# liuQuan98/APR

Measured on AMD Instinct MI355X. Metric: point-cloud pairs/sec (120k-pt KITTI frame, FCGF encode+match+SVD), higher is better.
Workload: dtype f32

## Files before the change

### apr_amd/_lib.py

```python
from __future__ import annotations

import ctypes as C
import os

import torch

_HERE = os.path.dirname(os.path.abspath(__file__))
LIB_PATH = os.path.join(_HERE, "lib", "libapr_hip.so")

_p = C.c_void_p
_i32, _i64, _u64, _f32, _f64, _sz = C.c_int32, C.c_int64, C.c_uint64, C.c_float, C.c_double, C.c_size_t

class PairDesc(C.Structure):
    _fields_ = [("f0", C.c_void_p), ("n0", C.c_int64), ("f1", C.c_void_p), ("n1", C.c_int64),
                ("xyz0", C.c_void_p), ("xyz1", C.c_void_p), ("seed", C.c_uint64)]


class SpconvDesc(C.Structure):
    _fields_ = [("inp", C.c_void_p), ("ldi", C.c_int64), ("nbr", C.c_void_p), ("n_out", C.c_int64),
                ("K", C.c_int32), ("cin", C.c_int32), ("cout", C.c_int32), ("relu", C.c_int32),
                ("w_packed", C.c_void_p), ("scale", C.c_void_p), ("shift", C.c_void_p),
                ("residual", C.c_void_p), ("ldr", C.c_int64), ("out", C.c_void_p), ("ldo", C.c_int64),
                ("counters", C.c_void_p), ("plist", C.c_void_p), ("prod_scratch", C.c_void_p),
                ("plist_bytes", C.c_int64), ("w_bf3", C.c_void_p),
# ... 86 lines not shown
    "apr_pairlist3_build": (C.c_int, [_p, _i64, _i32, _p, _p, _sz, _p]),
    "apr_spconv_ws3_supported": (C.c_int, [_i32, _i32, _i32]),
    "apr_spconv_ws3_fwd_bf3": (C.c_int, [_p, _i64, _p, _p, _i64, _i32, _i32, _p, _p, _p, _p, _i64, _i32, _p, _i64, _p, _p]),
    "apr_spconv_ws_fwd": (C.c_int, [_p, _i64, _p, _p, _i64, _i32, _i32, _i32, _p, _p, _p, _p, _i64, _i32, _p, _i64, _p, _p]),
    "apr_spconv_packed_bf3_bytes": (_i64, [_i32, _i32, _i32]),
    "apr_spconv_pack_weights_bf3": (C.c_int, [_p, _i32, _i32, _i32, _p, _p]),
    "apr_spconv_pack_weights_bf3_ex": (C.c_int, [_p, _i32, _i32, _i32, _i32, _i32, _p, _p]),
    "apr_spconv_ws_fwd_bf3": (C.c_int, [_p, _i64, _p, _p, _i64, _i32, _i32, _i32, _p, _p, _p, _p, _p, _i64, _i32, _p, _i64,
                                        _p, _p]),
    "apr_spconv_wgrad_scratch_bytes": (_sz, [_i64, _i32, _i32, _i32]),
    "apr_spconv_wgrad": (C.c_int, [_p, _i64, _p, _i64, _p, _i64, _i32, _i32, _i32, _p, _p, _sz, _p]),
    "apr_spconv_wgrad_same_level": (C.c_int, [_p, _i64, _p, _i64, _p, _i64, _i32, _i32, _i32, _p, _p, _sz, _p]),
    "apr_spconv_route": (_i32, [_p]),
    "apr_spconv_tile_variant": (_i32, [_p]),
    "apr_dense_gemm_bf3_variant": (_i32, [_i64, _i32, _i32]),
    "apr_spconv_wgrad_plan": (C.c_int, [_p, _i64, _p, _i64, _i64, _i32, _i32, _i32, _i32, _p]),
    "apr_spconv_ws_supported": (_i32, [_i32, _i32, _i32]),
    "apr_spconv_bigk_supported": (_i32, [_i32, _i32, _i32]),
    "apr_spconv_fwd_batch": (C.c_int, [_p, _i32, _p]),
    "apr_spconv_fwd_batch_timed": (C.c_int, [_p, _i32, _p, _p]),
    "apr_bn_stats": (C.c_int, [_p, _i64, _i64, _i32, _p, _p, _p, _sz, _p]),
    "apr_norm_params": (C.c_int, [_p, _i64, _i64, _i32, _f32, _p, _p, _p, _sz, _p]),
    "apr_bn_stats_scratch_bytes": (_sz, [_i64, _i32]),
    "apr_instance_norm_act": (C.c_int, [_p, _i64, _i64, _i32, _f32, _p, _i64, _i32, _f32, _p, _i64, _p, _sz, _p]),
    "apr_spconv_os_tile_rows": (_i32, [_i64, _i32, _i32]),
    "apr_spconv_os_pairs_bytes": (_sz, [_i64, _i32, _i32]),
    "apr_spconv_os_pairs_build": (C.c_int, [_p, _i64, _i64, _i32, _i32, _p, _sz, _p]),
    "apr_spconv_os_trace": (C.c_int, [_p, _i32]),
    "apr_spconv_os_set_debug": (C.c_int, [_i32]),
    "apr_spconv_os_fwd": (C.c_int, [_p, _i64, _p, _i64, _i32, _i32, _i32, _i32, _p, _p, _p, _p, _i64, _i32, _p, _i64, _p]),
    "apr_norm_backward_scratch_bytes": (_sz, [_i64, _i32]),
    "apr_norm_backward": (C.c_int, [_p, _i64, _p, _i64, _i64, _i32, _p, _p, _p, _p, _i64, _p, _p, _p, _sz, _p]),
    "apr_bn_train_fwd": (C.c_int, [_p, _i64, _i64, _i32, _p, _p, C.c_float, C.c_float, _p, _p, _p, _i64, _i32, _p, _i64, _p, _p,
                                   _p, _p, _i32, _p, _sz, _p]),
    "apr_bn_train_bwd": (C.c_int, [_p, _i64, _p, _i64, _p, _i64, _i64, _i32, _p, _p, _p, _i32, _p, _i64, _p, _i64, _p, _p,
                                   _p, _i32, _p, _sz, _p]),
    "apr_weights_flip_transpose": (C.c_int, [_p, _i32, _i32, _i32, _i32, _p, _p]),
    "apr_dense_gemm_bf3": (C.c_int, [_p, _i64, _i64, _i32, _i32, _p, _p, _p, _p, _i64, _i32, _p, _i64, _p]),
    "apr_dense_rows_bf3_ok": (_i32, [_i32, _i32]),
    "apr_dense_rows_bf3_route": (_i32, [_i64, _i32, _i32]),
    "apr_dense_rows_bf3": (C.c_int, [_p, _i64, _i64, _i32, _i32, _p, _p, _p, _p, _i64, _i32, _i32, _p, _i64, _p]),
    "apr_dense_gemm_bf3_norm_scratch_bytes": (_sz, [_i64, _i32, _i32]),
    "apr_dense_gemm_bf3_norm_act": (C.c_int, [_p, _i64, _i64, _i32, _i32, _p, _f32, _p, _i64, _i32, _f32, _p, _i64, _p, _i32, _p,
                                              _sz, _p]),
    "apr_weighted_choice_round": (C.c_int64, [_p, _i64, _p, _i64, _i64, _p, _i64, _p, _p, _i32]),
    "apr_instance_norm_act_seg": (C.c_int, [_p, _i64, _i64, _i32, _f32, _p, _i64, _i32, _f32, _p, _i64, _p, _i32, _p, _sz, _p]),
    "apr_affine_act": (C.c_int, [_p, _i64, _i64, _i32, _p, _p, _p, _i64, _i32, _f32, _p, _i64, _p]),
    "apr_act_backward": (C.c_int, [_p, _i64, _p, _i64, _i64, _i32, _i32, _f32, _p, _i64, _p]),
    "apr_l2_normalize": (C.c_int, [_p, _i64, _i64, _i32, _p, _i64, _p]),
    "apr_l2_normalize_backward": (C.c_int, [_p, _i64, _p, _i64, _i64, _i32, _p, _i64, _p]),
    "apr_feature_nn": (C.c_int, [_p, _i64, _p, _i64, _i32, _p, _p]),
    "apr_feature_nn_fast_scratch_bytes": (_sz, [_i64, _i64, _i32]),
    "apr_feature_nn_fast": (C.c_int, [_p, _i64, _p, _i64, _i32, _p, _p, _sz, _p]),
    "apr_nn_unpack": (C.c_int, [_p, _i64, _p, _p, _p]),
    "apr_ransac_scratch_bytes": (_sz, [_i64, _i64]),
    "apr_ransac_pose": (C.c_int, [_p, _i64, _p, _i64, _p, _f64, _f64, _i64, _u64, _p, _sz, _p, _p]),
    "apr_ransac_geometric_scratch_bytes": (_sz, [_i64, _i64, _i64]),
    "apr_ransac_pose_geometric": (C.c_int, [_p, _i64, _p, _i64, _p, _f64, _f64, _i64, _i64, _u64, _p, _sz, _p, _p]),
    "apr_ransac_raw_bytes": (_sz, []),
    "apr_ransac_pose_geometric_async": (C.c_int, [_p, _i64, _p, _i64, _p, _f64, _f64, _i64, _i64, _u64, _p, _sz, _p, _p]),
    "apr_ransac_decode": (C.c_int, [_p, _p]),
    "apr_ransac_pose_async": (C.c_int, [_p, _i64, _p, _i64, _p, _f64, _f64, _i64, _u64, _p, _sz, _p, _p]),
    "apr_fcgf_test_pair": (C.c_int, [_p, _i64, _p, _i64, _p, _p, _i64, _i64, _p, _p, _i64, _p, _i64, _p, _p, _p, _f64, _f64,
                                     _f64, _i64, _p, _p, _i64, _i64, _p]),
    "apr_irls_pose": (C.c_int, [_p, _p, _p, _i64, _p, _p, _sz, _p]),
    "apr_match_pose_batch_scratch_bytes": (_sz, [_i32, _i64, _i64, _i32, _i64]),
    "apr_match_pose_batch": (C.c_int, [_p, _i32, _i32, C.c_double, C.c_double, _i64, _p, _sz, _p, _p]),
    "apr_match_pose_batch_slot_bytes": (_sz, [_i32]),
    "apr_match_pose_set_lanes": (C.c_int, [_i32]),
    "apr_match_pose_batch_enqueue": (C.c_int, [_p, _i32, _i32, C.c_double, C.c_double, _i64, _p, _sz, _p, _p]),
    "apr_match_pose_batch_finish": (C.c_int, [_p, _i32, _i32, C.c_double, C.c_double, _i64, _p, _sz, _p, _p, _p]),
    "apr_irls_scratch_bytes": (_sz, [_i64]),
    "apr_valid_pair": (C.c_int, [_p, _i64, _p, _i64, _p, _p, _i64, _i64, _p, _p, _f32, _p, _i64, _i64, _p, _sz, _p]),
    "apr_valid_pair_scratch_bytes": (_sz, [_i64]),
    "apr_predator_valid_record": (C.c_int, [_p, _p, _p, _p, _p, _p, _p, _p, _i64, _i64, _p, _i64, _i64, _p]),
    "apr_predator_test_pair": (C.c_int, [_p, _i64, _p, _i64, _p, _p, _p, _p, _f64, _f64, _f64, _f64, _p, _i64, _i64, _p]),
    "apr_contrastive_reduce": (C.c_int, [_p, _p, _i32, _i32, _p, _p, _p, _p, _p, _p, _p, _i32, _i64, _f32, _f32, _p, _p]),
    "apr_pair_rows_from_nn": (C.c_int, [_p, _i64, _p, _i64, _p, _p]),
    "apr_pair_dist": (C.c_int, [_p, _i64, _p, _i64, _i32, _p, _p, _i64, _i64, _f32, _p, _p, _p, _p]),
    "apr_pair_terms_scratch_bytes": (_sz, [_i64]),
    "apr_pair_terms_reduce": (C.c_int, [_p, _p, _p, _i64, _p, _i64, _p, _i64, _i64, _f32, _i32, _p, _p, _p, _p, _p, _p, _sz, _p]),
    "apr_pair_grad_scratch_bytes": (_sz, [_i64, _i64, _i64]),
    "apr_pair_grad": (C.c_int, [_p, _i64, _p, _i64, _i32, _p, _p, _i64, _p, _p, _p, _p, _i32, _p, _p, _p, _sz, _p]),
    "apr_grid_subsample_scratch_bytes": (_sz, [_i64]),
    "apr_grid_subsample": (C.c_int, [_p, _i64, _p, _i32, _f32, _p, _i32, _p, _p, _p, _p, _sz, _p]),
    "apr_grid_subsample_async": (C.c_int, [_p, _i64, _p, _i32, _f32, _p, _i32, _p, _p, _p, _p, _sz, _p]),
    "apr_voxel_down_sample_scratch_bytes": (_sz, [_i64]),
    "apr_voxel_down_sample": (C.c_int, [_p, _i64, _p, _i32, _f64, _p, _p, _p, _p, _p, _p, _p, _sz, _p]),
    "apr_sample_augment": (C.c_int, [_p, _p, _i64, _f64, _p, _f64, _p, _p, _p]),
    "apr_cloud_mean": (C.c_int, [_p, _i64, _p, _p]),
    "apr_radius_scratch_bytes": (_sz, [_i64, _i64]),
    "apr_radius_neighbors_async": (C.c_int, [_p, _i64, _p, _i64, _p, _p, _i32, _f32, _i32, _p, _i64, _p, _p, _sz, _p]),
    "apr_radius_neighbors_regrid_async": (C.c_int, [_p, _i64, _p, _i64, _p, _p, _i32, _f32, _i32, _p, _i64, _p, _p, _sz, _p]),
    "apr_radius_neighbors": (C.c_int, [_p, _i64, _p, _i64, _p, _p, _i32, _f32, _i32, _p, _i64, _p, _p, _sz, _p]),
    "apr_knn": (C.c_int, [_p, _i32, _i32, _i32, _p, _p]),
    "apr_row_sums": (C.c_int, [_p, _i64, _i64, _i32, _p, _p]),
    "apr_kpconv_weighted": (C.c_int, [_p, _i64, _p, _i64, _p, _i32, _p, _i64, _i32, _p, _i32, _f32, _p, _p, _i64, _p]),
    "apr_kpconv_fused_ok": (_i32, [_i32, _i32, _i32]),
    "apr_kpconv_fused_route": (_i32, [_i64, _i32, _i32, _i32]),
    "apr_kpconv_fused": (C.c_int, [_p, _i64, _p, _i64, _p, _i32, _p, _i64, _i32, _p, _i32, _f32, _p, _p, _i32, _p, _i64, _p]),
    "apr_kpconv_dfeat": (C.c_int, [_p, _i64, _p, _i64, _p, _i32, _p, _i64, _i32, _p, _i32, _f32, _p, _p, _i64, _p]),
    "apr_kpconv_dfeat_contrib": (C.c_int, [_p, _i64, _p, _i64, _p, _i32, _p, _i64, _i32, _p, _i32, _f32, _p, _p, _p]),
    "apr_kpconv_deform_weighted": (C.c_int, [_p, _i64, _p, _i64, _p, _i32, _p, _i64, _i32, _p, _p, _i32, _f32, _p, _p, _i64, _p,
                                             _p]),
    "apr_kpconv_deform_dfeat_contrib": (C.c_int, [_p, _i64, _p, _i64, _p, _i32, _p, _i64, _i32, _p, _p, _i32, _f32, _p, _p, _p]),
    "apr_kpconv_deform_dgeom": (C.c_int, [_p, _i64, _p, _i64, _p, _i32, _p, _i64, _i32, _p, _i64, _p, _p, _i32, _f32, _p, _p, _p,
# ... 130 lines not shown
```

### apr_amd/csrc/match_mfma.hip

```cpp
#include "common.h"

namespace {

typedef float f32x4 __attribute__((ext_vector_type(4)));
typedef float f32x2 __attribute__((ext_vector_type(2)));
typedef __bf16 bf16x8 __attribute__((ext_vector_type(8)));

constexpr float kEpsRel = 1e-4f;
constexpr float kEpsAbs = 5e-5f;

__device__ inline unsigned short to_bf16_rne(float x) {
  unsigned u = __float_as_uint(x);
  u += 0x7FFFu + ((u >> 16) & 1u);
  return (unsigned short)(u >> 16);
}

template <int C>
__global__ void k_nn_prep(const float* __restrict__ f, int64_t n, float len_scale, float row_scale,
                          unsigned short* __restrict__ fb, unsigned short* __restrict__ fl, f32x4* __restrict__ meta,
                          unsigned* __restrict__ u_init, unsigned long long* __restrict__ best_init,
                          unsigned* __restrict__ zero_me) {
  constexpr int LPR = C / 4;
  const int64_t t = (int64_t)blockIdx.x * blockDim.x + threadIdx.x;
  const int64_t row = t / LPR;
// ... 315 lines not shown
    }
  }
  if (!REFINE && wave_live) {
#pragma unroll
    for (int qt = 0; qt < QT; ++qt)
#pragma unroll
      for (int r = 0; r < 4; ++r) {
        float v = mn[qt][r];
#pragma unroll
        for (int d = 1; d < 16; d <<= 1) v = fminf(v, __shfl_xor(v, d));
        const int64_t row = q0 + qt * 16 + lq * 4 + r;
        if (l16 == 0 && row < n0) {
          const f32x4 m = qmeta[row];
          const float u = fmaxf(v + m[1] + m[0] * len_max, 0.f);
          atomicMin(&U[row], __float_as_uint(u));
        }
      }
  }
}

template <int C>
__device__ inline void nn_tile_eval(float* my_t, const f32x4* xv, const float* __restrict__ f1, int64_t j0, int64_t j1,
                                    int lane, float& bd, int& bj) {
  constexpr int VPR = C / 4;
#pragma unroll
  for (int v = lane; v < 16 * VPR; v += 64) {
    const int r = v / VPR, g = v - r * VPR;
    const int64_t row = (j0 + r < j1) ? j0 + r : j1 - 1;
    *reinterpret_cast<f32x4*>(my_t + r * C + g * 4) = *reinterpret_cast<const f32x4*>(f1 + row * C + g * 4);
  }
#pragma unroll 2
  for (int jj = 0; jj < 16; ++jj) {
    float s0 = 0.f, s1 = 0.f, s2 = 0.f, s3 = 0.f;
#pragma unroll
    for (int g = 0; g < C / 4; ++g) {
      const f32x4 yv = *reinterpret_cast<const f32x4*>(my_t + jj * C + g * 4);
      const float d0 = xv[g][0] - yv[0], d1 = xv[g][1] - yv[1];
      const float d2 = xv[g][2] - yv[2], d3 = xv[g][3] - yv[3];
      s0 = fmaf(d0, d0, s0);
      s1 = fmaf(d1, d1, s1);
      s2 = fmaf(d2, d2, s2);
      s3 = fmaf(d3, d3, s3);
    }
    const float dd = (s0 + s1) + (s2 + s3);
    const int64_t j = (j0 + jj < j1) ? j0 + jj : j1 - 1;
    if (dd < bd) {
      bd = dd;
      bj = (int)j;
    }
  }
}

template <int C>
__global__ __launch_bounds__(256) void k_nn_resolve(const unsigned long long* __restrict__ cand,
                                                    const unsigned* __restrict__ cand_count, unsigned nwg, unsigned nexact,
                                                    const unsigned long long* __restrict__ shared_list,
                                                    const unsigned* __restrict__ overflow, unsigned shared_cap,
                                                    const unsigned* __restrict__ dense_list, int chunk, unsigned qwaves,
                                                    const float* __restrict__ f0, int64_t n0,
                                                    const float* __restrict__ f1, int64_t n1,
                                                    unsigned long long* __restrict__ best) {
  __shared__ __attribute__((aligned(16))) float s_t[4][16 * C];
  const int lane = threadIdx.x & 63;
  const int wave = __builtin_amdgcn_readfirstlane(threadIdx.x >> 6);
  if (overflow[0] != 0u) {
    const int64_t nqt = (n0 + 63) >> 6, ntt = (n1 + 15) >> 4;
    const int64_t nw = (int64_t)gridDim.x * 4;
    const int64_t slices = nw / nqt > 0 ? nw / nqt : 1;
    const int64_t tps = (ntt + slices - 1) / slices;
    for (int64_t w = (int64_t)blockIdx.x * 4 + wave; w < nqt * slices; w += nw) {
      const int64_t q = (w % nqt) * 64 + lane;
      const int64_t tt0 = (w / nqt) * tps, tt1 = min((long long)(tt0 + tps), (long long)ntt);
      const float* x = f0 + (q < n0 ? q : n0 - 1) * C;
      f32x4 xv[C / 4];
#pragma unroll
      for (int g = 0; g < C / 4; ++g) xv[g] = *reinterpret_cast<const f32x4*>(x + g * 4);
      float bd = __builtin_inff();
      int bj = 0x7fffffff;
      for (int64_t tt = tt0; tt < tt1; ++tt)
        nn_tile_eval<C>(s_t[wave], xv, f1, tt * 16, min((long long)(tt * 16 + 16), (long long)n1), lane, bd, bj);
      if (q < n0 && bj != 0x7fffffff) {
        const unsigned long long mine = ((unsigned long long)__float_as_uint(bd) << 32) | (unsigned)bj;
        if (mine < __builtin_nontemporal_load(&best[q])) atomicMin(&best[q], mine);
      }
    }
    return;
  }
  if (blockIdx.x < nexact) {
    const bool shared = blockIdx.x >= nwg;
    const unsigned wave_id = blockIdx.x * 4 + (threadIdx.x >> 6);
    const unsigned n = shared ? min(overflow[1], shared_cap) : min(cand_count[wave_id], (unsigned)kCandWave);
    const unsigned long long* src = shared ? shared_list : cand + (size_t)wave_id * kCandWave;
    const unsigned first = shared ? (blockIdx.x - nwg) * 256u + threadIdx.x : (threadIdx.x & 63u);
    const unsigned step = shared ? (nexact - nwg) * 256u : 64u;
    for (unsigned t = first; t < n; t += step) {
      const unsigned long long ij = src[t];
      const int64_t i = (int64_t)(ij >> 32), j = (int64_t)(ij & 0xffffffffull);
      const float* x = f0 + i * C;
      const float* y = f1 + j * C;
      float s0 = 0.f, s1 = 0.f, s2 = 0.f, s3 = 0.f;
#pragma unroll
      for (int g = 0; g < C / 4; ++g) {
        const f32x4 xv = *reinterpret_cast<const f32x4*>(x + g * 4);
        const f32x4 yv = *reinterpret_cast<const f32x4*>(y + g * 4);
        const float d0 = xv[0] - yv[0], d1 = xv[1] - yv[1], d2 = xv[2] - yv[2], d3 = xv[3] - yv[3];
        s0 = fmaf(d0, d0, s0);
        s1 = fmaf(d1, d1, s1);
        s2 = fmaf(d2, d2, s2);
        s3 = fmaf(d3, d3, s3);
      }
      const float d = (s0 + s1) + (s2 + s3);
      const unsigned long long mine = ((unsigned long long)__float_as_uint(d) << 32) | (unsigned)j;
      if (mine < __builtin_nontemporal_load(&best[i])) atomicMin(&best[i], mine);
    }
    return;
  }
  const unsigned tpc = (unsigned)chunk >> 4;
  const unsigned n = min(overflow[2], kDenseListCap);
  const unsigned nwaves = (gridDim.x - nexact) * 4;
  for (unsigned e = (blockIdx.x - nexact) * 4 + wave; e < n; e += nwaves) {
    const unsigned fb = __builtin_amdgcn_readfirstlane(dense_list[e]);
    const unsigned wave_id = fb / tpc, tile = fb % tpc;
    const unsigned dq = (wave_id % qwaves) * 64u;
    const unsigned t0 = (wave_id / qwaves) * (unsigned)chunk;
    const int64_t q = (int64_t)dq + lane;
    const int64_t j0 = (int64_t)t0 + (int64_t)tile * 16;
    const int64_t j1 = min(min((long long)(j0 + 16), (long long)((int64_t)t0 + chunk)), (long long)n1);
    const float* x = f0 + (q < n0 ? q : n0 - 1) * C;
    f32x4 xv[C / 4];
#pragma unroll
    for (int g = 0; g < C / 4; ++g) xv[g] = *reinterpret_cast<const f32x4*>(x + g * 4);
    float bd = __builtin_inff();
    int bj = 0x7fffffff;
    nn_tile_eval<C>(s_t[wave], xv, f1, j0, j1, lane, bd, bj);
    if (q < n0 && bj != 0x7fffffff) {
      const unsigned long long mine = ((unsigned long long)__float_as_uint(bd) << 32) | (unsigned)bj;
      if (mine < __builtin_nontemporal_load(&best[q])) atomicMin(&best[q], mine);
    }
  }
}

int64_t shared_capacity(int64_t n0) {
  int64_t c = 64 * n0;
  if (c < 65536) c = 65536;
  return c < (1ll << 31) ? c : (1ll << 31) - 1;
}

void nn_grid(int64_t n0, int64_t n1, int feat_c, int64_t* qblocks, int64_t* chunk, int64_t* nchunk) {
  static const int s_wgs = env_int("APR_NN_GRID_WGS", 768);
  static const int s_want = env_int("APR_NN_WANT", 0);
  *qblocks = cdiv64(n0, 256);
  int64_t want = cdiv64(s_wgs > 0 && s_wgs < 768 ? s_wgs : 768, *qblocks);
  if (feat_c >= 64) {
    const int64_t fit = 512 / *qblocks;
    if (fit >= 1 && fit < want) want = fit;
  }
  if (s_want > 0 && s_want <= want) want = s_want;
  int64_t c = cdiv64(cdiv64(n1, want), 64) * 64;
  if (c < 256) c = 256;
  if (c >= (1 << 24)) c = (1 << 24) - 64;
  *chunk = c;
  *nchunk = cdiv64(n1, c);
}

size_t dense_list_bytes(int64_t qblocks, int64_t nchunk, int64_t chunk) {
  uint64_t nflag = (uint64_t)(qblocks * 4) * (uint64_t)nchunk * (uint64_t)(chunk / 16);
  if (nflag > kDenseListCap) nflag = kDenseListCap;
  return apr_align256((size_t)nflag * 4 + 64);
}

template <int C>
int run_fast(const float* f0, int64_t n0, const float* f1, int64_t n1, unsigned long long* best, void* scratch,
             size_t scratch_bytes, hipStream_t st) {
  AprArena a(scratch);
  int64_t qblocks, chunk, nchunk;
  nn_grid(n0, n1, C, &qblocks, &chunk, &nchunk);
  const int64_t nwaves = qblocks * nchunk * 4;
  unsigned short* qb = a.take<unsigned short>((size_t)n0 * C);
  unsigned short* ql = a.take<unsigned short>((size_t)n0 * C);
  unsigned short* tb = a.take<unsigned short>((size_t)n1 * C);
  unsigned short* tl = a.take<unsigned short>((size_t)n1 * C);
  f32x4* qmeta = a.take<f32x4>(n0);
  f32x4* tmeta = a.take<f32x4>(n1);
  unsigned* U = a.take<unsigned>(n0);
  unsigned* overflow = a.take<unsigned>(64);
  unsigned* cand_count = a.take<unsigned>(nwaves);
  unsigned long long* cand = a.take<unsigned long long>((size_t)nwaves * kCandWave);
  unsigned long long* shared_list = a.take<unsigned long long>(shared_capacity(n0));
  a.take<char>((size_t)(qblocks * 4) * (size_t)nchunk * (size_t)(chunk / 16) + 64);
  unsigned* dense_list = (unsigned*)a.take<char>(dense_list_bytes(qblocks, nchunk, chunk));
  APR_CHECK_ARG(a.fits(scratch_bytes), "apr_feature_nn_fast: scratch too small");
  const unsigned shared_cap = (unsigned)shared_capacity(n0);
  constexpr int LPR = C / 4;
  if ((uint64_t)qblocks * 4 * (uint64_t)nchunk * (uint64_t)(chunk / 16) + 64 >= (1ull << 32)) {
    apr_set_error("apr_feature_nn_fast: problem too large for the dense-block ids");
    return APR_EINVAL;
  }
  hipLaunchKernelGGL((k_nn_prep2<C>), dim3((unsigned)cdiv64((n0 + n1) * LPR, 256)), dim3(256), 0, st, f0, n0, f1, n1, qb, ql,
                     qmeta, tb, tl, tmeta, U, best, overflow);
  static const int s_dense_min = env_int("APR_NN_DENSE_MIN", kDenseMin);
  static const int s_bound_div = env_int("APR_NN_BOUND_DIV", 4);
  const dim3 grid((unsigned)qblocks, (unsigned)nchunk);
  hipLaunchKernelGGL((k_nn_mfma<C, false>), grid, dim3(256), 0, st, qb, ql, qmeta, n0, tb, tl, tmeta, n1, (int)chunk, U,
                     cand, cand_count, overflow, shared_list, shared_cap, dense_list, overflow + 2, s_bound_div);
  hipLaunchKernelGGL((k_nn_mfma<C, true>), grid, dim3(256), 0, st, qb, ql, qmeta, n0, tb, tl, tmeta, n1, (int)chunk, U,
                     cand, cand_count, overflow, shared_list, shared_cap, dense_list, overflow + 2, s_dense_min);
  const unsigned nwg = (unsigned)(qblocks * nchunk);
  const unsigned nexact = nwg + 256;
  hipLaunchKernelGGL((k_nn_resolve<C>), dim3(nexact + 1024), dim3(256), 0, st, cand, cand_count, nwg, nexact, shared_list,
                     overflow, shared_cap, dense_list, (int)chunk, (unsigned)(qblocks * 4), f0, n0, f1, n1, best);
  APR_LAUNCH_CHECK();
  return APR_OK;
}

}

APR_API size_t apr_feature_nn_fast_scratch_bytes(int64_t n0, int64_t n1, int32_t c) {
  if (n0 < 0 || n1 < 0 || c <= 0) return 0;
  if (n0 < 1) n0 = 1;
  if (n1 < 1) n1 = 1;
  const size_t qblocks = (size_t)cdiv64(n0, 256);
  const size_t nwaves = 4 * (768 + qblocks);
  const size_t nflag = qblocks * 4 * ((2 * (size_t)n1 + 320) / 16 + 1);
  const size_t nlist = nflag > kDenseListCap ? (size_t)kDenseListCap : nflag;
  const auto al = apr_align256;
  return 2 * al((size_t)n0 * c * 2) + 2 * al((size_t)n1 * c * 2) + al((size_t)n0 * 16) + al((size_t)n1 * 16) +
         al((size_t)n0 * 4) + 256 + al(nwaves * 4) + al(nwaves * kCandWave * 8) +
         al((size_t)shared_capacity(n0) * 8) + al(nflag + 64) + al(nlist * 4 + 64) + 512;
}

APR_API int apr_feature_nn_fast(const float* f0, int64_t n0, const float* f1, int64_t n1, int32_t c, uint64_t* best,
                                void* scratch, size_t scratch_bytes, void* stream) {
  hipStream_t st = (hipStream_t)stream;
  APR_CHECK_ARG(n0 >= 0 && n1 > 0 && n1 < (1ll << 31) && n0 < (1ll << 31), "apr_feature_nn_fast: bad shape");
  APR_CHECK_ARG(c == 32 || c == 64 || c == 128, "apr_feature_nn_fast: c=%d, supported: 32, 64, 128", c);
  APR_CHECK_ARG(n1 < (1ll << 24) - 64, "apr_feature_nn_fast: n1 = %lld, supported below 2^24 - 64 targets", (long long)n1);
  APR_CHECK_ARG(((((uintptr_t)f0) | ((uintptr_t)f1)) & 15) == 0, "apr_feature_nn_fast: 16-byte aligned rows required");
  APR_CHECK_ARG(scratch_bytes >= apr_feature_nn_fast_scratch_bytes(n0, n1, c), "apr_feature_nn_fast: scratch too small");
  if (n0 == 0) return APR_OK;
  unsigned long long* b = (unsigned long long*)best;
  if (c == 32) return run_fast<32>(f0, n0, f1, n1, b, scratch, scratch_bytes, st);
  if (c == 64) return run_fast<64>(f0, n0, f1, n1, b, scratch, scratch_bytes, st);
  return run_fast<128>(f0, n0, f1, n1, b, scratch, scratch_bytes, st);
}
```

### apr_amd/ops.py

```python
from __future__ import annotations

import ctypes as C
import os

import numpy as np
import torch

from . import _lib
from ._lib import check, ptr, stream


def _lib_():
    return _lib.load()


def _f32(t, name):
    if not t.is_cuda or t.dtype != torch.float32:
        raise _lib.AprHipError(f"{name}: need a float32 GPU tensor (no CPU fallback), got {t.dtype} on {t.device}")
    return t


def _rows(t, name):
    _f32(t, name)
    if t.dim() != 2 or (t.shape[1] > 1 and t.stride(1) != 1):
# ... 969 lines not shown
    def backward(ctx, dy, _dm, _dv):
        x, mean, rstd, weight = ctx.saved_tensors
        g = None if weight is None else weight.reshape(-1).contiguous()
        dx, dg, db = norm_backward(x, dy.contiguous(), mean, rstd, g, want_affine_grads=weight is not None or ctx.has_bias)
        dw = dg.reshape(weight.shape) if weight is not None else None
        dbias = db if ctx.has_bias else None
        return dx, dw, dbias, None


def affine_act(x, scale=None, shift=None, residual=None, relu=False, out=None, leaky=None):
    x, ldx = _rows(x, "affine_act.x")
    n, c = x.shape
    if out is None:
        out = torch.empty((n, c), dtype=torch.float32, device=x.device)
    out, ldy = _rows(out, "affine_act.out")
    ldr = 0
    if residual is not None:
        residual, ldr = _rows(residual, "affine_act.residual")
    mode = 2 if leaky is not None else int(bool(relu))
    check(_lib_().apr_affine_act(ptr(x), ldx, n, c, ptr(scale), ptr(shift), ptr(residual), ldr, mode,
                                 float(leaky or 0.0), ptr(out), ldy, stream()))
    return out


def l2_normalize(x, out=None):
    x, ldx = _rows(x, "l2_normalize.x")
    n, c = x.shape
    if out is None:
        out = torch.empty((n, c), dtype=torch.float32, device=x.device)
    out, ldy = _rows(out, "l2_normalize.out")
    check(_lib_().apr_l2_normalize(ptr(x), ldx, n, c, ptr(out), ldy, stream()))
    return out


class L2NormalizeFunction(torch.autograd.Function):

    @staticmethod
    def forward(ctx, x):
        x = x.contiguous()
        ctx.save_for_backward(x)
        return l2_normalize(x)

    @staticmethod
    def backward(ctx, dy):
        (x,) = ctx.saved_tensors
        dy = dy.contiguous()
        n, c = x.shape
        dx = torch.empty_like(x)
        check(_lib_().apr_l2_normalize_backward(ptr(x), c, ptr(dy), c, n, c, ptr(dx), c, stream()))
        return dx



def feature_nn(f0, f1, return_distance=False, impl=None):
    f0 = _f32(f0, "feature_nn.f0").contiguous()
    f1 = _f32(f1, "feature_nn.f1").contiguous()
    if f0.shape[1] != f1.shape[1]:
        raise _lib.AprHipError("feature_nn: channel mismatch")
    n0, c = f0.shape
    n1 = f1.shape[0]
    lib = _lib_()
    best = torch.empty(n0, dtype=torch.int64, device=f0.device)
    if impl is None:
        impl = os.environ.get("APR_NN_IMPL", "fast")
    if impl not in ("brute", "fast"):
        raise _lib.AprHipError(f"feature_nn: unknown impl {impl!r}")
    if impl == "fast" and c in (32, 64, 128):
        sb = int(lib.apr_feature_nn_fast_scratch_bytes(n0, n1, c))
        scratch = torch.empty(sb, dtype=torch.uint8, device=f0.device)
        check(lib.apr_feature_nn_fast(ptr(f0), n0, ptr(f1), n1, c, ptr(best), ptr(scratch), sb, stream()))
    else:
        check(lib.apr_feature_nn(ptr(f0), n0, ptr(f1), n1, c, ptr(best), stream()))
    idx = torch.empty(n0, dtype=torch.int64, device=f0.device)
    d2 = torch.empty(n0, dtype=torch.float32, device=f0.device) if return_distance else None
    check(lib.apr_nn_unpack(ptr(best), n0, ptr(idx), ptr(d2), stream()))
    return (idx, d2) if return_distance else idx



def _dev(t, dtype, name):
    if not torch.is_tensor(t) or not t.is_cuda or t.dtype != dtype:
        raise _lib.AprHipError(f"{name}: need a {dtype} GPU tensor (no CPU fallback), got "
                               f"{getattr(t, 'dtype', type(t))} on {getattr(t, 'device', 'the host')}")
    return t.contiguous()


def overlap_labels(correspondence, n_src, n_tgt):
    corr = _dev(correspondence, torch.int64, "overlap_labels.correspondence")
    dev = corr.device
    gt = torch.empty(n_src + n_tgt, dtype=torch.float32, device=dev)
    src_idx = torch.empty(n_src, dtype=torch.int32, device=dev)
    tgt_idx = torch.empty(n_tgt, dtype=torch.int32, device=dev)
    counts = torch.empty(3, dtype=torch.int32, device=dev)
    check(_lib_().apr_overlap_labels(ptr(corr), corr.shape[0], n_src, n_tgt, ptr(gt), ptr(src_idx), ptr(tgt_idx), ptr(counts),
                                     stream()))
    return gt, src_idx, tgt_idx, counts


def weighted_bce(pred, gt, n_dev=None):
    pred, gt = _dev(pred, torch.float32, "weighted_bce.pred"), _dev(gt, torch.float32, "weighted_bce.gt")
    if pred.dim() != 1 or pred.shape != gt.shape:
        raise _lib.AprHipError("weighted_bce: prediction and gt must be vectors of one length")
    lib = _lib_()
    sb = int(lib.apr_weighted_bce_scratch_bytes())
    scratch = torch.empty(sb, dtype=torch.uint8, device=pred.device)
    out = torch.empty(8, dtype=torch.float32, device=pred.device)
    check(lib.apr_weighted_bce_forward(ptr(pred), ptr(gt), pred.shape[0], ptr(n_dev), ptr(out), ptr(scratch), sb, stream()))
    return out


def weighted_bce_backward(pred, gt, out8, grad_out, n_dev=None, scatter_pos=None, dpred=None):
    pred, gt = _dev(pred, torch.float32, "weighted_bce_backward.pred"), _dev(gt, torch.float32, "weighted_bce_backward.gt")
    out8, grad_out = _dev(out8, torch.float32, "weighted_bce_backward.out8"), _dev(grad_out, torch.float32, "weighted_bce_backward.grad_out")
    if dpred is None:
        dpred = torch.zeros_like(pred)
    check(_lib_().apr_weighted_bce_backward(ptr(pred), ptr(gt), pred.shape[0], ptr(n_dev), ptr(out8), ptr(grad_out),
                                            ptr(scatter_pos), ptr(dpred), stream()))
    return dpred


def gathered_argmax(a, a_idx, na_dev, b, b_idx, nb_dev):
    a, b = _dev(a, torch.float32, "gathered_argmax.a"), _dev(b, torch.float32, "gathered_argmax.b")
    a_idx, b_idx = _dev(a_idx, torch.int32, "gathered_argmax.a_idx"), _dev(b_idx, torch.int32, "gathered_argmax.b_idx")
    if a.dim() != 2 or b.dim() != 2 or a.shape[1] != b.shape[1]:
        raise _lib.AprHipError("gathered_argmax: channel mismatch")
    row_arg = torch.zeros(a_idx.shape[0], dtype=torch.int32, device=a.device)
    col_arg = torch.zeros(b_idx.shape[0], dtype=torch.int32, device=a.device)
    check(_lib_().apr_gathered_argmax(ptr(a), ptr(a_idx), ptr(na_dev), a_idx.shape[0], ptr(b), ptr(b_idx), ptr(nb_dev),
                                      b_idx.shape[0], a.shape[1], ptr(row_arg), ptr(col_arg), stream()))
# ... 806 lines not shown
```

### include/apr_hip.h

```cpp
#ifndef APR_HIP_H
#define APR_HIP_H

#include <stddef.h>
#include <stdint.h>

#ifdef __cplusplus
extern "C" {
#endif

#define APR_OK 0
#define APR_EINVAL (-1)
#define APR_EHIP (-2)
#define APR_ETIMEOUT (-3)
#define APR_ERANGE (-3)

const char* apr_last_error(void);
int apr_version(void);
int apr_device_count(void);
int32_t apr_struct_sizes(int32_t* out, int32_t n);
int apr_event_wait(void* event, int32_t poll_us);
int apr_event_wait_timeout(void* event, int32_t poll_us, int64_t timeout_us);


int64_t apr_hash_capacity(int64_t n);
// ... 187 lines not shown
                      void* arena, size_t arena_bytes, apr_pyramid* out, void* stream);


int apr_bn_stats(const float* x, int64_t ld, int64_t n, int32_t c,
                 float* mean, float* var, void* scratch, size_t scratch_bytes, void* stream);
size_t apr_bn_stats_scratch_bytes(int64_t n, int32_t c);

size_t apr_norm_backward_scratch_bytes(int64_t n, int32_t c);
int apr_norm_backward(const float* x, int64_t ldx, const float* dy, int64_t lddy, int64_t n, int32_t c,
                      const float* mean, const float* rstd, const float* gamma, float* dx, int64_t lddx,
                      float* dgamma, float* dbeta, void* scratch, size_t scratch_bytes, void* stream);

int apr_bn_train_fwd(const float* z, int64_t ldz, int64_t n, int32_t c, const float* gamma, const float* beta,
                     float eps, float momentum, float* running_mean, float* running_var, const float* residual,
                     int64_t ldr, int32_t relu, float* y, int64_t ldy, float* save_mean, float* save_rstd,
                     int64_t* num_batches_tracked, const int64_t* seg_offsets_host, int32_t nseg, void* scratch,
                     size_t scratch_bytes, void* stream);
int apr_bn_train_bwd(const float* z, int64_t ldz, const float* y, int64_t ldy, const float* dy, int64_t lddy,
                     int64_t n, int32_t c, const float* mean, const float* rstd, const float* gamma, int32_t relu,
                     float* dx, int64_t lddx, float* dres, int64_t lddres, float* dgamma, float* dbeta,
                     const int64_t* seg_offsets_host, int32_t nseg, void* scratch, size_t scratch_bytes, void* stream);

int apr_col_sums(const float* x, int64_t ld, int64_t n, int32_t c, float* sums, void* scratch, size_t scratch_bytes,
                 void* stream);

int apr_norm_params(const float* x, int64_t ld, int64_t n, int32_t c, float eps, float* scale, float* shift,
                    void* scratch, size_t scratch_bytes, void* stream);

int apr_instance_norm_act(const float* x, int64_t ldx, int64_t n, int32_t c, float eps, const float* residual,
                          int64_t ldr, int32_t relu, float negative_slope, float* y, int64_t ldy, void* scratch,
                          size_t scratch_bytes, void* stream);
int apr_instance_norm_act_seg(const float* x, int64_t ldx, int64_t n, int32_t c, float eps, const float* residual,
                              int64_t ldr, int32_t relu, float negative_slope, float* y, int64_t ldy,
                              const int64_t* seg_offsets_host, int32_t nseg, void* scratch, size_t scratch_bytes,
                              void* stream);

int apr_affine_act(const float* x, int64_t ldx, int64_t n, int32_t c,
                   const float* scale, const float* shift,
                   const float* residual, int64_t ldr, int32_t relu, float negative_slope,
                   float* y, int64_t ldy, void* stream);
int apr_act_backward(const float* dy, int64_t lddy, const float* y, int64_t ldy, int64_t n, int32_t c, int32_t mode,
                     float negative_slope, float* dz, int64_t lddz, void* stream);

int apr_l2_normalize(const float* x, int64_t ldx, int64_t n, int32_t c,
                     float* y, int64_t ldy, void* stream);
int apr_l2_normalize_backward(const float* x, int64_t ldx, const float* dy, int64_t lddy, int64_t n, int32_t c,
                              float* dx, int64_t lddx, void* stream);

int apr_feature_nn(const float* f0, int64_t n0, const float* f1, int64_t n1, int32_t c,
                   uint64_t* best, void* stream);
size_t apr_feature_nn_fast_scratch_bytes(int64_t n0, int64_t n1, int32_t c);
int apr_feature_nn_fast(const float* f0, int64_t n0, const float* f1, int64_t n1, int32_t c, uint64_t* best,
                        void* scratch, size_t scratch_bytes, void* stream);
int apr_nn_unpack(const uint64_t* best, int64_t n, int64_t* idx, float* d2, void* stream);

size_t apr_ransac_scratch_bytes(int64_t n0, int64_t max_iter);
int apr_ransac_pose(const float* xyz0, int64_t n0, const float* xyz1, int64_t n1,
                    const int64_t* corr, double max_dist, double edge_ratio,
                    int64_t max_iter, uint64_t seed,
                    void* scratch, size_t scratch_bytes, double* result_host, void* stream);

size_t apr_ransac_geometric_scratch_bytes(int64_t n0, int64_t n1, int64_t max_iter);
int apr_ransac_pose_geometric(const float* xyz0, int64_t n0, const float* xyz1, int64_t n1,
                              const int64_t* corr, double max_dist, double edge_ratio,
                              int64_t max_iter, int64_t max_validation, uint64_t seed,
                              void* scratch, size_t scratch_bytes, double* result_host, void* stream);
size_t apr_ransac_raw_bytes(void);
int apr_ransac_pose_geometric_async(const float* xyz0, int64_t n0, const float* xyz1, int64_t n1,
                                    const int64_t* corr, double max_dist, double edge_ratio, int64_t max_iter,
                                    int64_t max_validation, uint64_t seed, void* scratch, size_t scratch_bytes,
                                    void* raw_dev, void* stream);
int apr_ransac_decode(const void* raw_host, double* result_host);
int apr_ransac_pose_async(const float* xyz0, int64_t n0, const float* xyz1, int64_t n1, const int64_t* corr,
                          double max_dist, double edge_ratio, int64_t max_iter, uint64_t seed, void* scratch,
                          size_t scratch_bytes, void* raw_dev, void* stream);

typedef struct {
  const float* f0; int64_t n0;
  const float* f1; int64_t n1;
  const float* xyz0;
  const float* xyz1;
  uint64_t seed;
} apr_pair_desc;
size_t apr_match_pose_batch_scratch_bytes(int32_t B, int64_t n0_max, int64_t n1_max, int32_t c, int64_t max_iter);
int apr_match_pose_batch(const apr_pair_desc* pairs, int32_t B, int32_t c, double max_dist, double edge_ratio,
                         int64_t max_iter, void* scratch, size_t scratch_bytes, double* results_host, void* stream);
size_t apr_match_pose_batch_slot_bytes(int32_t B);
int apr_match_pose_batch_enqueue(const apr_pair_desc* pairs, int32_t B, int32_t c, double max_dist, double edge_ratio,
                                 int64_t max_iter, void* scratch, size_t scratch_bytes, void* slots_host, void* stream);
int apr_match_pose_batch_finish(const apr_pair_desc* pairs, int32_t B, int32_t c, double max_dist, double edge_ratio,
                                int64_t max_iter, void* scratch, size_t scratch_bytes, const void* slots_host,
                                double* results_host, void* stream);

int apr_ransac_set_screen(int32_t mode);
int apr_ransac_set_option(int32_t option, int32_t value);
int apr_ransac_sampling_launches(int64_t* out2);

int apr_match_pose_set_lanes(int32_t lanes);

int apr_irls_pose(const float* pts0, const float* pts1, const float* weight, int64_t n,
                  float* T_host, void* scratch, size_t scratch_bytes, void* stream);
size_t apr_irls_scratch_bytes(int64_t n);

#define APR_VALID_RECORD_FLOATS 24
int apr_valid_pair(const float* xyz0, int64_t n0, const float* xyz1, int64_t n1, const int64_t* sel0,
                   const int64_t* sel1, int64_t m0, int64_t m1, const int64_t* nn, const float* T_gt,
// ... 326 lines not shown
```

Baseline: 2783.

## Resolve NN candidates with row-cooperative coalesced loads staged through LDS

Adds a row-cooperative resolve path for the feature nearest-neighbour candidate lists. Lanes now load slices of several candidate rows with coalesced vector loads, write the differences to per-wave LDS, and each lane then reduces one candidate's distance. The old path had one lane gather a whole row on its own. The new path is on by default when a list holds enough candidates. It adds an env override, a counts diagnostic kernel, reusable scratch, and larger LDS use per block, which may lower occupancy.

```diff
diff --git a/apr_amd/_lib.py b/apr_amd/_lib.py
--- a/apr_amd/_lib.py
+++ b/apr_amd/_lib.py
@@ -162,6 +162,7 @@
     "apr_feature_nn": (C.c_int, [_p, _i64, _p, _i64, _i32, _p, _p]),
     "apr_feature_nn_fast_scratch_bytes": (_sz, [_i64, _i64, _i32]),
     "apr_feature_nn_fast": (C.c_int, [_p, _i64, _p, _i64, _i32, _p, _p, _sz, _p]),
+    "apr_feature_nn_fast_counts": (C.c_int, [_p, _i64, _i64, _i32, _p, _p]),
     "apr_nn_unpack": (C.c_int, [_p, _i64, _p, _p, _p]),
     "apr_ransac_scratch_bytes": (_sz, [_i64, _i64]),
     "apr_ransac_pose": (C.c_int, [_p, _i64, _p, _i64, _p, _f64, _f64, _i64, _u64, _p, _sz, _p, _p]),
diff --git a/apr_amd/csrc/match_mfma.hip b/apr_amd/csrc/match_mfma.hip
--- a/apr_amd/csrc/match_mfma.hip
+++ b/apr_amd/csrc/match_mfma.hip
@@ -391,6 +391,89 @@
 }
 
 template <int C>
+__device__ inline void nn_cand_lanes(const unsigned long long* __restrict__ src, unsigned first, unsigned n, unsigned step,
+                                     const float* __restrict__ f0, const float* __restrict__ f1,
+                                     unsigned long long* __restrict__ best) {
+  for (unsigned t = first; t < n; t += step) {
+    const unsigned long long ij = src[t];
+    const int64_t i = (int64_t)(ij >> 32), j = (int64_t)(ij & 0xffffffffull);
+    const float* x = f0 + i * C;
+    const float* y = f1 + j * C;
+    float s0 = 0.f, s1 = 0.f, s2 = 0.f, s3 = 0.f;
+#pragma unroll
+    for (int g = 0; g < C / 4; ++g) {
+      const f32x4 xv = *reinterpret_cast<const f32x4*>(x + g * 4);
+      const f32x4 yv = *reinterpret_cast<const f32x4*>(y + g * 4);
+      const float d0 = xv[0] - yv[0], d1 = xv[1] - yv[1], d2 = xv[2] - yv[2], d3 = xv[3] - yv[3];
+      s0 = fmaf(d0, d0, s0);
+      s1 = fmaf(d1, d1, s1);
+      s2 = fmaf(d2, d2, s2);
+      s3 = fmaf(d3, d3, s3);
+    }
+    const float d = (s0 + s1) + (s2 + s3);
+    const unsigned long long mine = ((unsigned long long)__float_as_uint(d) << 32) | (unsigned)j;
+    if (mine < __builtin_nontemporal_load(&best[i])) atomicMin(&best[i], mine);
+  }
+}
+
+constexpr int kRowsStage = 2048;
+constexpr int kRowsStagePad = kRowsStage + 4 * 64;
+
+template <int C>
+__device__ inline void nn_cand_rows(float* __restrict__ st, const unsigned long long* __restrict__ src, unsigned first,
+                                    unsigned n, unsigned step, const float* __restrict__ f0,
+                                    const float* __restrict__ f1, unsigned long long* __restrict__ best, int lane) {
+  constexpr int LPR = C / 4;
+  constexpr int B = kRowsStage / C;
+  constexpr int RPP = 64 / LPR;
+  constexpr int NP = B / RPP;
+  constexpr int LD = C + 4;
+  const int sub = lane / LPR, g = lane - sub * LPR;
+  if (first >= n) return;
+  auto word = [&](unsigned b0) {
+    const unsigned nb = min(n - b0, (unsigned)B);
+    return src[b0 + min((unsigned)lane, nb - 1u)];
+  };
+  unsigned long long w = word(first);
+  for (unsigned b0 = first; b0 < n; b0 += step) {
+    const unsigned nb = min(n - b0, (unsigned)B);
+    const unsigned wi = (unsigned)(w >> 32), wj = (unsigned)w;
+    f32x4 xv[NP], yv[NP];
+#pragma unroll
+    for (int p = 0; p < NP; ++p) {
+      const int64_t i = (int64_t)(unsigned)__shfl((int)wi, p * RPP + sub);
+      const int64_t j = (int64_t)(unsigned)__shfl((int)wj, p * RPP + sub);
+      xv[p] = *reinterpret_cast<const f32x4*>(f0 + i * C + g * 4);
+      yv[p] = *reinterpret_cast<const f32x4*>(f1 + j * C + g * 4);
+    }
+    const unsigned nxt = b0 + step;
+    unsigned long long wn = 0ull;
+    if (nxt < n) wn = word(nxt);
+    asm volatile("" ::: "memory");
+#pragma unroll
+    for (int p = 0; p < NP; ++p)
+      *reinterpret_cast<f32x4*>(st + (p * RPP + sub) * LD + g * 4) = xv[p] - yv[p];
+    asm volatile("" ::: "memory");
+    if ((unsigned)lane < nb) {
+      const float* d = st + lane * LD;
+      float s0 = 0.f, s1 = 0.f, s2 = 0.f, s3 = 0.f;
+#pragma unroll
+      for (int gg = 0; gg < C / 4; ++gg) {
+        const f32x4 dv = *reinterpret_cast<const f32x4*>(d + gg * 4);
+        s0 = fmaf(dv[0], dv[0], s0);
+        s1 = fmaf(dv[1], dv[1], s1);
+        s2 = fmaf(dv[2], dv[2], s2);
+        s3 = fmaf(dv[3], dv[3], s3);
+      }
+      const float dd = (s0 + s1) + (s2 + s3);
+      const unsigned long long mine = ((unsigned long long)__float_as_uint(dd) << 32) | wj;
+      if (mine < __builtin_nontemporal_load(&best[wi])) atomicMin(&best[wi], mine);
+    }
+    w = wn;
+  }
+}
+
+template <int C, bool ROWS>
 __global__ __launch_bounds__(256) void k_nn_resolve(const unsigned long long* __restrict__ cand,
                                                     const unsigned* __restrict__ cand_count, unsigned nwg, unsigned nexact,
                                                     const unsigned long long* __restrict__ shared_list,
@@ -398,8 +481,10 @@
                                                     const unsigned* __restrict__ dense_list, int chunk, unsigned qwaves,
                                                     const float* __restrict__ f0, int64_t n0,
                                                     const float* __restrict__ f1, int64_t n1,
-                                                    unsigned long long* __restrict__ best) {
-  __shared__ __attribute__((aligned(16))) float s_t[4][16 * C];
+                                                    unsigned long long* __restrict__ best, unsigned rows_min) {
+  constexpr int kWaveLds = ROWS ? kRowsStagePad : 16 * C;
+  static_assert(kWaveLds >= 16 * C && (!ROWS || kWaveLds >= (kRowsStage / C) * (C + 4)), "per-wave LDS too small");
+  __shared__ __attribute__((aligned(16))) float s_t[4][kWaveLds];
   const int lane = threadIdx.x & 63;
   const int wave = __builtin_amdgcn_readfirstlane(threadIdx.x >> 6);
   if (overflow[0] != 0u) {
@@ -430,27 +515,15 @@
     const unsigned wave_id = blockIdx.x * 4 + (threadIdx.x >> 6);
     const unsigned n = shared ? min(overflow[1], shared_cap) : min(cand_count[wave_id], (unsigned)kCandWave);
     const unsigned long long* src = shared ? shared_list : cand + (size_t)wave_id * kCandWave;
-    const unsigned first = shared ? (blockIdx.x - nwg) * 256u + threadIdx.x : (threadIdx.x & 63u);
-    const unsigned step = shared ? (nexact - nwg) * 256u : 64u;
-    for (unsigned t = first; t < n; t += step) {
-      const unsigned long long ij = src[t];
-      const int64_t i = (int64_t)(ij >> 32), j = (int64_t)(ij & 0xffffffffull);
-      const float* x = f0 + i * C;
-      const float* y = f1 + j * C;
-      float s0 = 0.f, s1 = 0.f, s2 = 0.f, s3 = 0.f;
-#pragma unroll
-      for (int g = 0; g < C / 4; ++g) {
-        const f32x4 xv = *reinterpret_cast<const f32x4*>(x + g * 4);
-        const f32x4 yv = *reinterpret_cast<const f32x4*>(y + g * 4);
-        const float d0 = xv[0] - yv[0], d1 = xv[1] - yv[1], d2 = xv[2] - yv[2], d3 = xv[3] - yv[3];
-        s0 = fmaf(d0, d0, s0);
-        s1 = fmaf(d1, d1, s1);
-        s2 = fmaf(d2, d2, s2);
-        s3 = fmaf(d3, d3, s3);
-      }
-      const float d = (s0 + s1) + (s2 + s3);
-      const unsigned long long mine = ((unsigned long long)__float_as_uint(d) << 32) | (unsigned)j;
-      if (mine < __builtin_nontemporal_load(&best[i])) atomicMin(&best[i], mine);
+    if (ROWS && n >= rows_min) {
+      constexpr unsigned B = kRowsStage / C;
+      const unsigned first = shared ? ((blockIdx.x - nwg) * 4u + (unsigned)wave) * B : 0u;
+      const unsigned step = shared ? (nexact - nwg) * 4u * B : B;
+      nn_cand_rows<C>(s_t[wave], src, first, n, step, f0, f1, best, lane);
+    } else {
+      const unsigned first = shared ? (blockIdx.x - nwg) * 256u + threadIdx.x : (threadIdx.x & 63u);
+      const unsigned step = shared ? (nexact - nwg) * 256u : 64u;
+      nn_cand_lanes<C>(src, first, n, step, f0, f1, best);
     }
     return;
   }
@@ -508,26 +581,69 @@
   return apr_align256((size_t)nflag * 4 + 64);
 }
 
+struct NnScratch {
+  int64_t qblocks, chunk, nchunk, nwaves;
+  unsigned short *qb, *ql, *tb, *tl;
+  f32x4 *qmeta, *tmeta;
+  unsigned *U, *overflow, *cand_count, *dense_list;
+  unsigned long long *cand, *shared_list;
+};
+
+NnScratch nn_carve(AprArena& a, int64_t n0, int64_t n1, int c) {
+  NnScratch s;
+  nn_grid(n0, n1, c, &s.qblocks, &s.chunk, &s.nchunk);
+  s.nwaves = s.qblocks * s.nchunk * 4;
+  s.qb = a.take<unsigned short>((size_t)n0 * c);
+  s.ql = a.take<unsigned short>((size_t)n0 * c);
+  s.tb = a.take<unsigned short>((size_t)n1 * c);
+  s.tl = a.take<unsigned short>((size_t)n1 * c);
+  s.qmeta = a.take<f32x4>(n0);
+  s.tmeta = a.take<f32x4>(n1);
+  s.U = a.take<unsigned>(n0);
+  s.overflow = a.take<unsigned>(64);
+  s.cand_count = a.take<unsigned>(s.nwaves);
+  s.cand = a.take<unsigned long long>((size_t)s.nwaves * kCandWave);
+  s.shared_list = a.take<unsigned long long>(shared_capacity(n0));
+  a.take<char>((size_t)(s.qblocks * 4) * (size_t)s.nchunk * (size_t)(s.chunk / 16) + 64);
+  s.dense_list = (unsigned*)a.take<char>(dense_list_bytes(s.qblocks, s.nchunk, s.chunk));
+  return s;
+}
+
+__global__ __launch_bounds__(256) void k_nn_counts(const unsigned* __restrict__ cand_count, int64_t nwaves,
+                                                   const unsigned* __restrict__ overflow, unsigned shared_cap,
+                                                   unsigned long long* __restrict__ counts) {
+  __shared__ unsigned long long s_sum[4];
+  unsigned long long s = 0;
+  for (int64_t w = threadIdx.x; w < nwaves; w += 256) s += min(cand_count[w], (unsigned)kCandWave);
+#pragma unroll
+  for (int d = 32; d >= 1; d >>= 1) s += __shfl_xor(s, d);
+  if ((threadIdx.x & 63) == 0) s_sum[threadIdx.x >> 6] = s;
+  __syncthreads();
+  if (threadIdx.x == 0) {
+    counts[0] = (s_sum[0] + s_sum[1]) + (s_sum[2] + s_sum[3]);
+    counts[1] = min(overflow[1], shared_cap);
+    counts[2] = overflow[2];
+  }
+}
+
+bool nn_resolve_rows() {
+  static const bool s_rows = [] {
+    const char* v = getenv("APR_NN_RESOLVE");
+    return !(v && strcmp(v, "lanes") == 0);
+  }();
+  return s_rows;
+}
+
 template <int C>
 int run_fast(const float* f0, int64_t n0, const float* f1, int64_t n1, unsigned long long* best, void* scratch,
              size_t scratch_bytes, hipStream_t st) {
   AprArena a(scratch);
-  int64_t qblocks, chunk, nchunk;
-  nn_grid(n0, n1, C, &qblocks, &chunk, &nchunk);
-  const int64_t nwaves = qblocks * nchunk * 4;
-  unsigned short* qb = a.take<unsigned short>((size_t)n0 * C);
-  unsigned short* ql = a.take<unsigned short>((size_t)n0 * C);
-  unsigned short* tb = a.take<unsigned short>((size_t)n1 * C);
-  unsigned short* tl = a.take<unsigned short>((size_t)n1 * C);
-  f32x4* qmeta = a.take<f32x4>(n0);
-  f32x4* tmeta = a.take<f32x4>(n1);
-  unsigned* U = a.take<unsigned>(n0);
-  unsigned* overflow = a.take<unsigned>(64);
-  unsigned* cand_count = a.take<unsigned>(nwaves);
-  unsigned long long* cand = a.take<unsigned long long>((size_t)nwaves * kCandWave);
-  unsigned long long* shared_list = a.take<unsigned long long>(shared_capacity(n0));
-  a.take<char>((size_t)(qblocks * 4) * (size_t)nchunk * (size_t)(chunk / 16) + 64);
-  unsigned* dense_list = (unsigned*)a.take<char>(dense_list_bytes(qblocks, nchunk, chunk));
+  const NnScratch s = nn_carve(a, n0, n1, C);
+  const int64_t qblocks = s.qblocks, chunk = s.chunk, nchunk = s.nchunk;
+  unsigned short *qb = s.qb, *ql = s.ql, *tb = s.tb, *tl = s.tl;
+  f32x4 *qmeta = s.qmeta, *tmeta = s.tmeta;
+  unsigned *U = s.U, *overflow = s.overflow, *cand_count = s.cand_count, *dense_list = s.dense_list;
+  unsigned long long *cand = s.cand, *shared_list = s.shared_list;
   APR_CHECK_ARG(a.fits(scratch_bytes), "apr_feature_nn_fast: scratch too small");
   const unsigned shared_cap = (unsigned)shared_capacity(n0);
   constexpr int LPR = C / 4;
@@ -546,8 +662,16 @@
                      cand, cand_count, overflow, shared_list, shared_cap, dense_list, overflow + 2, s_dense_min);
   const unsigned nwg = (unsigned)(qblocks * nchunk);
   const unsigned nexact = nwg + 256;
-  hipLaunchKernelGGL((k_nn_resolve<C>), dim3(nexact + 1024), dim3(256), 0, st, cand, cand_count, nwg, nexact, shared_list,
-                     overflow, shared_cap, dense_list, (int)chunk, (unsigned)(qblocks * 4), f0, n0, f1, n1, best);
+  static const int s_rows_min = env_int("APR_NN_ROWS_MIN", -1);
+  const int rows_min = s_rows_min >= 0 ? s_rows_min : kRowsStage / C / 2;
+  if (nn_resolve_rows())
+    hipLaunchKernelGGL((k_nn_resolve<C, true>), dim3(nexact + 1024), dim3(256), 0, st, cand, cand_count, nwg, nexact,
+                       shared_list, overflow, shared_cap, dense_list, (int)chunk, (unsigned)(qblocks * 4), f0, n0, f1, n1,
+                       best, (unsigned)rows_min);
+  else
+    hipLaunchKernelGGL((k_nn_resolve<C, false>), dim3(nexact + 1024), dim3(256), 0, st, cand, cand_count, nwg, nexact,
+                       shared_list, overflow, shared_cap, dense_list, (int)chunk, (unsigned)(qblocks * 4), f0, n0, f1, n1,
+                       best, (unsigned)rows_min);
   APR_LAUNCH_CHECK();
   return APR_OK;
 }
@@ -582,3 +706,16 @@
   if (c == 64) return run_fast<64>(f0, n0, f1, n1, b, scratch, scratch_bytes, st);
   return run_fast<128>(f0, n0, f1, n1, b, scratch, scratch_bytes, st);
 }
+
+APR_API int apr_feature_nn_fast_counts(const void* scratch, int64_t n0, int64_t n1, int32_t c, uint64_t* counts,
+                                       void* stream) {
+  APR_CHECK_ARG(n0 > 0 && n1 > 0 && n1 < (1ll << 24) - 64 && n0 < (1ll << 31), "apr_feature_nn_fast_counts: bad shape");
+  APR_CHECK_ARG(c == 32 || c == 64 || c == 128, "apr_feature_nn_fast_counts: c=%d, supported: 32, 64, 128", c);
+  APR_CHECK_ARG(scratch && counts, "apr_feature_nn_fast_counts: null pointer");
+  AprArena a(const_cast<void*>(scratch));
+  const NnScratch s = nn_carve(a, n0, n1, c);
+  hipLaunchKernelGGL(k_nn_counts, dim3(1), dim3(256), 0, (hipStream_t)stream, s.cand_count, s.nwaves, s.overflow,
+                     (unsigned)shared_capacity(n0), (unsigned long long*)counts);
+  APR_LAUNCH_CHECK();
+  return APR_OK;
+}
diff --git a/apr_amd/ops.py b/apr_amd/ops.py
--- a/apr_amd/ops.py
+++ b/apr_amd/ops.py
@@ -1045,7 +1045,7 @@
 
 
 
-def feature_nn(f0, f1, return_distance=False, impl=None):
+def feature_nn(f0, f1, return_distance=False, impl=None, scratch=None):
     f0 = _f32(f0, "feature_nn.f0").contiguous()
     f1 = _f32(f1, "feature_nn.f1").contiguous()
     if f0.shape[1] != f1.shape[1]:
@@ -1060,7 +1060,10 @@
         raise _lib.AprHipError(f"feature_nn: unknown impl {impl!r}")
     if impl == "fast" and c in (32, 64, 128):
         sb = int(lib.apr_feature_nn_fast_scratch_bytes(n0, n1, c))
-        scratch = torch.empty(sb, dtype=torch.uint8, device=f0.device)
+        if scratch is None:
+            scratch = torch.empty(sb, dtype=torch.uint8, device=f0.device)
+        elif scratch.dtype != torch.uint8 or scratch.device != f0.device or scratch.numel() < sb:
+            raise _lib.AprHipError(f"feature_nn: scratch must be a uint8 tensor of >= {sb} bytes on {f0.device}")
         check(lib.apr_feature_nn_fast(ptr(f0), n0, ptr(f1), n1, c, ptr(best), ptr(scratch), sb, stream()))
     else:
         check(lib.apr_feature_nn(ptr(f0), n0, ptr(f1), n1, c, ptr(best), stream()))
@@ -1068,6 +1071,16 @@
     d2 = torch.empty(n0, dtype=torch.float32, device=f0.device) if return_distance else None
     check(lib.apr_nn_unpack(ptr(best), n0, ptr(idx), ptr(d2), stream()))
     return (idx, d2) if return_distance else idx
+
+
+def feature_nn_scratch(n0, n1, c, device):
+    return torch.empty(int(_lib_().apr_feature_nn_fast_scratch_bytes(n0, n1, c)), dtype=torch.uint8, device=device)
+
+
+def feature_nn_counts(scratch, n0, n1, c):
+    counts = torch.empty(3, dtype=torch.int64, device=scratch.device)
+    check(_lib_().apr_feature_nn_fast_counts(ptr(scratch), n0, n1, c, ptr(counts), stream()))
+    return counts
 
 
 
diff --git a/include/apr_hip.h b/include/apr_hip.h
--- a/include/apr_hip.h
+++ b/include/apr_hip.h
@@ -263,6 +263,7 @@
 size_t apr_feature_nn_fast_scratch_bytes(int64_t n0, int64_t n1, int32_t c);
 int apr_feature_nn_fast(const float* f0, int64_t n0, const float* f1, int64_t n1, int32_t c, uint64_t* best,
                         void* scratch, size_t scratch_bytes, void* stream);
+int apr_feature_nn_fast_counts(const void* scratch, int64_t n0, int64_t n1, int32_t c, uint64_t* counts, void* stream);
 int apr_nn_unpack(const uint64_t* best, int64_t n, int64_t* idx, float* d2, void* stream);
 
 size_t apr_ransac_scratch_bytes(int64_t n0, int64_t max_iter);
```

Result: no change. 2776 (-0.2%).
